# bd-iaas-us/infiniStore

Measured on AMD Instinct MI355X. Metric: put_get_GBps, higher is better.
Workload: dtype bf16; 1 GPU; model=kvcache-store, block_kb=128, global_batch=2048, seq_len=0, parallelism=shard1, client_procs=4, resident_steps=976

## Files before the change

### csrc/server/server.cpp

```cpp
#include "server.h"

#include "../core/crash.h"

#include <algorithm>
#include <chrono>
#include <cstring>
#include <future>
#include <unistd.h>

#include "../core/log.h"

namespace ifs {

namespace {

bool debug_on() {
    static const bool on = getenv("IFS_SERVER_DEBUG") != nullptr;
    return on;
}
using Clock = std::chrono::steady_clock;
double us(Clock::time_point a, Clock::time_point b) {
    return std::chrono::duration<double, std::micro>(b - a).count();
}

// ... 365 lines not shown
            conn_close(c);
            return;
        }
    } else {
        uv_tcp_init(&io->loop, &c->tcp);
        c->tcp.data = c;
        if (uv_tcp_open(&c->tcp, fd) != 0) {
            conn_close(c);
            return;
        }
        uv_tcp_nodelay(&c->tcp, 1);
    }
    io->conns.push_back(c);
    uv_read_start(
        c->stream(),
        [](uv_handle_t*, size_t suggested, uv_buf_t* buf) {
            buf->base = static_cast<char*>(malloc(suggested));
            buf->len = suggested;
        },
        [](uv_stream_t* stream, ssize_t nread, const uv_buf_t* buf) {
            auto* c = static_cast<Conn*>(stream->data);
            Server* srv = c->srv;
            if (nread < 0) {
                free(buf->base);
                auto& v = c->owner->conns;
                v.erase(std::remove(v.begin(), v.end(), c), v.end());
                srv->verbs_teardown(c);
                srv->shm_teardown(c);
                conn_close(c);
                return;
            }
            if (nread == 0) {
                free(buf->base);
                return;
            }
            c->buf.insert(c->buf.end(), reinterpret_cast<uint8_t*>(buf->base),
                          reinterpret_cast<uint8_t*>(buf->base) + nread);
            free(buf->base);
            size_t consumed = 0;
            for (;;) {
                if (c->state == Conn::kHeader) {
                    if (c->buf.size() - consumed < sizeof(Header)) break;
                    memcpy(&c->hdr, c->buf.data() + consumed, sizeof(Header));
                    consumed += sizeof(Header);
                    if (c->hdr.magic != kMagic) {
                        WARN("bad magic from client; closing");
                        auto& v = c->owner->conns;
                        v.erase(std::remove(v.begin(), v.end(), c), v.end());
                        srv->verbs_teardown(c);
                        srv->shm_teardown(c);
                        conn_close(c);
                        return;
                    }
                    size_t cap = (c->hdr.op == OP_TCP_PUT) ? (256u << 20) : kProtocolBufferSize;
                    if (c->hdr.body_size > cap) {
                        WARN("body too large (%u) for op %c", c->hdr.body_size, c->hdr.op);
                        auto& v = c->owner->conns;
                        v.erase(std::remove(v.begin(), v.end(), c), v.end());
                        srv->verbs_teardown(c);
                        srv->shm_teardown(c);
                        conn_close(c);
                        return;
                    }
                    c->state = Conn::kBody;
                }
                if (c->state == Conn::kBody) {
                    if (c->buf.size() - consumed < c->hdr.body_size) break;
                    std::vector<uint8_t> body(c->buf.data() + consumed,
                                              c->buf.data() + consumed + c->hdr.body_size);
                    consumed += c->hdr.body_size;
                    c->state = Conn::kHeader;
                    srv->handle_request(c, c->hdr.op, std::move(body));
                    if (c->closed) return;
                }
            }
            if (consumed) c->buf.erase(c->buf.begin(), c->buf.begin() + consumed);
        });
}

namespace {

Server::LocalView to_view(const LocalMetaMsg& msg) {
    Server::LocalView v;
    v.device = msg.device;
    v.pid = msg.pid;
    v.base_ptr = msg.base_ptr;
    v.base_offset = msg.base_offset;
    v.block_size = msg.block_size;
    v.ipc = msg.ipc_handle.data();
    v.ipc_len = msg.ipc_handle.size();
    v.blocks.reserve(msg.blocks.size());
    for (auto& b : msg.blocks) v.blocks.push_back({std::string_view(b.key), b.offset});
    return v;
}

bool parse_packed_local(const uint8_t* body, size_t body_len, Server::LocalView* v) {
    if (body_len < sizeof(PackedLocalHdr)) return false;
    PackedLocalHdr h;
    memcpy(&h, body, sizeof(h));
    size_t n = h.n_blocks;
    size_t off_end = sizeof(h) + n * 8;
    if (body_len < off_end) return false;
    v->device = h.device;
    v->pid = h.pid;
    v->base_ptr = h.base_ptr;
    v->base_offset = h.base_offset;
    v->block_size = h.block_size;
    v->flags = h.flags;
    v->alloc_mb = h.rsvd;
    v->ipc = body + offsetof(PackedLocalHdr, ipc);
    v->ipc_len = 64;
    const uint64_t* offs = reinterpret_cast<const uint64_t*>(body + sizeof(h));
    const char* kp = reinterpret_cast<const char*>(body + off_end);
    const char* kend = reinterpret_cast<const char*>(body + body_len);
    v->blocks.reserve(n);
    for (size_t i = 0; i < n; i++) {
        const char* nul = static_cast<const char*>(memchr(kp, 0, kend - kp));
        const char* ke = nul ? nul : kend;
        if (kp > kend || (i + 1 < n && !nul)) return false;
        v->blocks.push_back({std::string_view(kp, ke - kp), offs[i]});
        kp = nul ? nul + 1 : kend;
    }
    return true;
}

}

void Server::handle_request(Conn* c, char op, std::vector<uint8_t> body) {
    DEBUG("request op=%s body=%zu", op_name(op).c_str(), body.size());
    struct Timer {
        Server* s;
        char op;
        std::chrono::steady_clock::time_point t0 = std::chrono::steady_clock::now();
        ~Timer() {
            auto us = std::chrono::duration_cast<std::chrono::microseconds>(
                          std::chrono::steady_clock::now() - t0)
                          .count();
            auto& st = s->op_stats_[static_cast<uint8_t>(op) & 127];
            st.count.fetch_add(1, std::memory_order_relaxed);
            st.total_us.fetch_add(static_cast<uint64_t>(us), std::memory_order_relaxed);
            uint64_t prev = st.max_us.load(std::memory_order_relaxed);
            while (static_cast<uint64_t>(us) > prev &&
                   !st.max_us.compare_exchange_weak(prev, static_cast<uint64_t>(us))) {
            }
        }
    } timer{this, op};
    switch (op) {
        case OP_W: {
            LocalMetaMsg msg;
            if (!parse_local_meta(body.data(), body.size(), &msg)) return send_status(c, INVALID_REQ);
            return op_local_write(c, to_view(msg), ReqCtx{});
        }
        case OP_R: {
            LocalMetaMsg msg;
            if (!parse_local_meta(body.data(), body.size(), &msg)) return send_status(c, INVALID_REQ);
            return op_local_read(c, to_view(msg), ReqCtx{});
        }
        case OP_W_FAST: {
            LocalView v;
            if (!parse_packed_local(body.data(), body.size(), &v))
                return send_status(c, INVALID_REQ);
            return op_local_write(c, v, ReqCtx{});
        }
        case OP_R_FAST: {
            LocalView v;
            if (!parse_packed_local(body.data(), body.size(), &v))
                return send_status(c, INVALID_REQ);
            return op_local_read(c, v, ReqCtx{});
        }
        case OP_SYNC:
            return op_sync(c, ReqCtx{});
        case OP_SHM_SETUP:
            return op_shm_setup(c, body);
        case OP_RDMA_EXCHANGE:
            return op_exchange(c, body);
        case OP_RDMA_ALLOCATE: {
            RemoteMetaMsg msg;
            if (!parse_remote_meta(body.data(), body.size(), &msg))
                return send_status(c, INVALID_REQ);
            return op_allocate(c, msg);
        }
        case OP_TCP_PUT:
            return op_tcp_put(c, std::move(body));
        case OP_TCP_GET: {
            RemoteMetaMsg msg;
            if (!parse_remote_meta(body.data(), body.size(), &msg))
                return send_status(c, INVALID_REQ);
            return op_tcp_get(c, msg);
        }
        case OP_RDMA_WRITE_COMMIT: {
            RemoteMetaMsg msg;
            if (!parse_remote_meta(body.data(), body.size(), &msg))
                return send_status(c, INVALID_REQ);
            return op_commit(c, msg);
        }
        case OP_CHECK_EXIST:
            return op_check_exist(c, body, ReqCtx{});
        case OP_GET_MATCH_LAST_IDX:
            return op_match_index(c, body, ReqCtx{});
        case OP_DELETE:
            return op_delete(c, body, ReqCtx{});
        case OP_STATS: {
            std::string js = stats_json();
            return send_status_payload(c, FINISH,
                                       reinterpret_cast<const uint8_t*>(js.data()), js.size());
        }
        default:
            WARN("unknown op '%c'", op);
            return send_status(c, INVALID_REQ);
    }
}

Shard* Server::shard_for_device(int device) {
    for (auto& s : shards_)
        if (s->device() == device) return s.get();
    return shards_[static_cast<size_t>(device < 0 ? 0 : device) % shards_.size()].get();
}

Shard* Server::shard_least_used() {
    Shard* best = shards_[0].get();
    size_t best_used = SIZE_MAX;
    for (auto& s : shards_) {
        size_t used = s->used_blocks();
        if (used < best_used) {
            best_used = used;
            best = s.get();
        }
    }
    return best;
}

void Server::maybe_extend(Shard* s) {
    if (!s->need_extend()) return;
    int expect = 0;
    if (!extending_.compare_exchange_strong(expect, 1)) return;
    std::lock_guard<std::mutex> jl(extend_mu_);
    if (extend_thread_.joinable()) extend_thread_.join();
    extend_thread_ = std::thread([this, s] {
        INFO("extending pool on shard dev=%d", s->device());
        void* arena = nullptr;
        if (s->extend(&arena) && arena) {
            std::lock_guard<std::mutex> lk(vdrv_mu_);
            if (vdrv_ && !vdrv_->reg_region(arena, opt_.extend_bytes, s->on_gpu(), nullptr))
                ERROR("MR registration of extended arena failed; verbs reads from it will error");
        }
        extending_.store(0);
    });
}

namespace {
void* resolve_client_base(Server::Conn* c, const Server::LocalView& msg) {
    if (msg.pid != 0 && msg.pid == static_cast<int32_t>(getpid()) && msg.base_ptr != 0)
        return reinterpret_cast<void*>(msg.base_ptr);
    if (msg.alloc_mb >= 2048) {
        ERROR("refusing IPC import of a %u MB client allocation: "
              "hipIpcOpenMemHandle hangs for >= 2 GiB allocations under "
              "dmabuf IPC; split the tensor or use the fabric path",
              msg.alloc_mb);
        return nullptr;
    }
    std::vector<uint8_t> key(msg.ipc, msg.ipc + msg.ipc_len);
    std::lock_guard<std::mutex> lk(c->ipc_mu);
    auto it = c->ipc_cache.find(key);
    if (it != c->ipc_cache.end()) return it->second.first;
    if (c->ipc_cache.size() >= 64 && c->remain.load() == 0 &&
        c->fabric_inflight.load() == 0 && c->ipc_pin.load() == 1) {
        for (auto& kv2 : c->ipc_cache) gpu::ipc_close(kv2.second.first);
        c->ipc_cache.clear();
    }
    gpu::IpcHandle h;
    memcpy(h.bytes, msg.ipc, gpu::kIpcHandleSize);
    void* base = gpu::ipc_open(h, msg.device);
    if (base) c->ipc_cache.emplace(std::move(key), std::make_pair(base, msg.device));
    return base;
}

struct IpcPinGuard {
    Server::Conn* c;
    explicit IpcPinGuard(Server::Conn* conn) : c(conn) { c->ipc_pin.fetch_add(1); }
    ~IpcPinGuard() { c->ipc_pin.fetch_sub(1); }
};
}

void Server::op_local_write(Conn* c, const LocalView& msg, const ReqCtx& ctx) {
    const bool dbg = debug_on();
    auto p0 = Clock::now();
    if (!gpu::available()) return reply_local(c, ctx, SYSTEM_ERROR);
    if (msg.ipc_len != gpu::kIpcHandleSize || msg.block_size <= 0)
        return reply_local(c, ctx, INVALID_REQ);
    IpcPinGuard pin(c);
    void* base = resolve_client_base(c, msg);
    if (!base) return reply_local(c, ctx, INTERNAL_ERROR);
    uint8_t* client_ptr = static_cast<uint8_t*>(base) + msg.base_offset;

    Shard* shard = shard_for_device(msg.device);
    size_t page = static_cast<size_t>(msg.block_size);
    size_t nb = msg.blocks.size();
    const bool quant = (msg.flags & kLocalFlagQuantFp8) != 0;
    if (quant && (page % 16 != 0)) return reply_local(c, ctx, INVALID_REQ);
    const size_t stored = quant ? page / 2 : page;

    std::vector<uint64_t> hashes(nb);
    for (size_t i = 0; i < nb; i++) hashes[i] = KvIndex::hash_of(msg.blocks[i].first);
    std::vector<uint32_t> fresh;
    fresh.reserve(nb);
    KvIndex::SweepTimes ta, td;
    index_.for_each_batched<KvIndex::Lock::kShared>(
        nb, hashes.data(), KvIndex::rotated_start(hashes.data(), nb),
        [&](KvMap& m, size_t i) {
            if (!index_.find_live(m, msg.blocks[i].first, hashes[i]))
                fresh.push_back(static_cast<uint32_t>(i));
            return true;
        },
        dbg ? &ta : nullptr);
    if (dbg && nb > 64)
        fprintf(stderr, "[pdbg2] dedup lockwait=%.0f underlock=%.0f\n", ta.lock_wait_us,
                ta.under_lock_us);
    auto p1 = Clock::now();

    n_writes_.fetch_add(1);
    size_t n_fresh = fresh.size();
    bytes_in_.fetch_add(n_fresh * page);
    bool sync_resp = (msg.flags & kLocalFlagSyncResponse) != 0;
    if (n_fresh == 0) {
        if (ctx.shm && !sync_resp) return;
        return reply_local(c, ctx, sync_resp ? FINISH : TASK_ACCEPTED);
    }

    std::vector<std::pair<void*, int>> slots;
    slots.reserve(n_fresh);
    auto try_alloc = [&] {
        slots.clear();
        return shard->allocate(stored, n_fresh,
                               [&](void* p, int idx) { slots.push_back({p, idx}); });
    };
    bool alloc_ok = try_alloc();
    for (int attempt = 0; !alloc_ok && opt_.auto_evict && attempt < 4; attempt++) {
        if (index_.evict_lru(shard, page * n_fresh * 2) == 0) break;
        alloc_ok = try_alloc();
    }
    if (!alloc_ok) return reply_local(c, ctx, OUT_OF_MEMORY);
    auto p2 = Clock::now();

    uint64_t t = index_.tick();
    SlabBatch slab_batch(n_fresh);
    auto entries = std::make_shared<std::vector<Ref<BlockEntry>>>();
    entries->reserve(n_fresh);
    Shard::CopyJob job;
    job.bytes_per_block = page;
    job.src.reserve(n_fresh);
    job.dst.reserve(n_fresh);
    auto scales_out =
        quant ? std::make_shared<std::vector<float>>(n_fresh, 1.f) : nullptr;
    if (quant) {
        job.xform = Shard::CopyJob::Xform::kQuantBf16Fp8;
        job.scales_out = scales_out;
    }
    for (size_t i = 0; i < n_fresh; i++) {
        auto* e = slab_batch.make();
        e->ptr = slots[i].first;
        e->size = stored;
        e->pool_idx = slots[i].second;
        e->shard = shard;
        e->committed = false;
        e->fp8 = quant;
        e->born_sec = KvIndex::now_sec();
        e->last_access.store(t, std::memory_order_relaxed);
        entries->emplace_back(e);
        job.src.push_back(
            reinterpret_cast<uint64_t>(client_ptr + msg.blocks[fresh[i]].second));
        job.dst.push_back(reinterpret_cast<uint64_t>(slots[i].first));
    }
    maybe_extend(shard);

    c->remain.fetch_add(1);
    c->ref();
    auto t_start = Clock::now();
    auto won = std::make_shared<std::vector<uint8_t>>(n_fresh, 0);
    auto copy_ok = std::make_shared<std::atomic<bool>>(false);
    auto arrivals = std::make_shared<std::atomic<int>>(0);
    auto fin = [this, c, entries, won, sync_resp, ctx, scales_out, copy_ok] {
        bool ok = copy_ok->load(std::memory_order_acquire);
        if (ok) {
            for (size_t i = 0; i < entries->size(); i++)
                if ((*won)[i]) {
                    if (scales_out) (*entries)[i]->scale = (*scales_out)[i];
                    (*entries)[i]->committed = true;
                }
        } else {
            c->ref();
            c->owner->post([this, c, entries, won] {
                std::vector<Ref<BlockEntry>> winners;
                for (size_t i = 0; i < entries->size(); i++)
                    if ((*won)[i]) winners.push_back((*entries)[i]);
                index_.erase_entries(winners);
                c->unref();
            });
        }
        if (sync_resp) reply_local(c, ctx, ok ? FINISH : INTERNAL_ERROR);
        finish_task(c, !ctx.shm);
    };
    job.done = [this, c, entries, fin, ctx, copy_ok, arrivals, t_start, dbg](bool ok) {
        if (dbg && entries->size() > 64)
            fprintf(stderr, "[sdbg] write n=%zu submit->complete=%.0fus\n", entries->size(),
                    us(t_start, Clock::now()));
        copy_ok->store(ok, std::memory_order_release);
        if (ctx.shm) {
            if (arrivals->fetch_add(1, std::memory_order_acq_rel) == 1) fin();
        } else {
            c->owner->post([fin, arrivals] {
                if (arrivals->fetch_add(1, std::memory_order_acq_rel) == 1) fin();
            });
        }
    };
    if (!sync_resp && !ctx.shm) send_status(c, TASK_ACCEPTED);
    bool submitted = shard->submit_copy(std::move(job));
    auto p2b = Clock::now();

    {
        std::vector<uint64_t> fresh_hashes(n_fresh);
        for (size_t p = 0; p < n_fresh; p++) fresh_hashes[p] = hashes[fresh[p]];
        std::vector<Ref<BlockEntry>> displaced;
        index_.for_each_batched<KvIndex::Lock::kExclusive>(
            n_fresh, fresh_hashes.data(), KvIndex::rotated_start(fresh_hashes.data(), n_fresh),
            [&](KvMap& m, size_t p) {
                (*won)[p] = index_.insert_locked(m, msg.blocks[fresh[p]].first, fresh_hashes[p],
                                                 (*entries)[p], true,
                                                 &displaced);
                return true;
            },
            dbg ? &td : nullptr);
        if (dbg && n_fresh > 64)
            fprintf(stderr, "[pdbg2] insert lockwait=%.0f underlock=%.0f\n", td.lock_wait_us,
                    td.under_lock_us);
    }
    if (submitted && arrivals->fetch_add(1, std::memory_order_acq_rel) == 1) fin();
    auto p3 = Clock::now();
    if (dbg && n_fresh > 64)
        fprintf(stderr, "[pdbg] dedup=%.0f alloc=%.0f submit=%.0f insert=%.0f\n", us(p0, p1),
                us(p1, p2), us(p2, p2b), us(p2b, p3));
    if (!submitted) {
        if (sync_resp) reply_local(c, ctx, INTERNAL_ERROR);
        finish_task(c, !ctx.shm);
    }
}

void Server::op_local_read(Conn* c, const LocalView& msg, const ReqCtx& ctx) {
    if (!gpu::available()) return reply_local(c, ctx, SYSTEM_ERROR);
    if (msg.ipc_len != gpu::kIpcHandleSize || msg.block_size <= 0)
        return reply_local(c, ctx, INVALID_REQ);
    IpcPinGuard pin(c);
    void* base = resolve_client_base(c, msg);
    if (!base) return reply_local(c, ctx, INTERNAL_ERROR);
    uint8_t* client_ptr = static_cast<uint8_t*>(base) + msg.base_offset;
    size_t page = static_cast<size_t>(msg.block_size);

    auto tr0 = Clock::now();
    static const bool cross_pull = [] {
        const char* v = getenv("IFS_CROSS_COPY");
        return v && std::string(v) == "reader";
    }();
    Shard* reader_shard = nullptr;
    if (cross_pull) {
        Shard* s = shard_for_device(msg.device);
        if (s->device() == msg.device) reader_shard = s;
    }
    auto exec_shard = [&](Shard* owner) {
        return (reader_shard && owner->device() != msg.device) ? reader_shard : owner;
    };
    std::map<Shard*, Shard::CopyJob> jobs;
    std::map<Shard*, Shard::CopyJob> qjobs;
    auto held = std::make_shared<std::vector<Ref<BlockEntry>>>();
    held->reserve(msg.blocks.size());
    uint64_t read_tick = index_.tick();
    std::vector<uint64_t> hashes(msg.blocks.size());
    for (size_t i = 0; i < hashes.size(); i++) hashes[i] = KvIndex::hash_of(msg.blocks[i].first);
    int err = 0;
    index_.for_each_batched<KvIndex::Lock::kShared>(
        hashes.size(), hashes.data(), 0, [&](KvMap& m, size_t i) {
            auto& b = msg.blocks[i];
            Ref<BlockEntry>* v = index_.find_live(m, b.first, hashes[i]);
            if (!v || !(*v)->committed) {
                err = KEY_NOT_FOUND;
                return false;
            }
            BlockEntry* e = v->get();
            e->last_access.store(read_tick, std::memory_order_relaxed);
            if (e->fp8 && e->size * 2 != page) {
                err = INVALID_REQ;
                return false;
            }
            auto& job = (e->fp8 ? qjobs : jobs)[exec_shard(e->shard)];
            job.bytes_per_block = page;
            if (e->fp8) {
                job.xform = Shard::CopyJob::Xform::kDequantFp8Bf16;
                job.scales_in.push_back(e->scale);
            }
            job.src.push_back(reinterpret_cast<uint64_t>(e->ptr));
            job.dst.push_back(reinterpret_cast<uint64_t>(client_ptr + b.second));
            held->push_back(*v);
            return true;
        });
    if (err) return reply_local(c, ctx, err);
    const bool dbg = debug_on();
    auto tcol = Clock::now();
    n_reads_.fetch_add(1);
    bytes_out_.fetch_add(msg.blocks.size() * page);
    bool sync_resp = (msg.flags & kLocalFlagSyncResponse) != 0;
    if (jobs.empty() && qjobs.empty())
        return reply_local(c, ctx, sync_resp ? FINISH : TASK_ACCEPTED);

    c->remain.fetch_add(1);
    c->ref();
    auto pending =
        std::make_shared<std::atomic<int>>(static_cast<int>(jobs.size() + qjobs.size()));
    auto all_ok = std::make_shared<std::atomic<bool>>(true);
    auto submit_one = [&](Shard* shard, Shard::CopyJob& job) -> bool {
        Shard::CopyJob j = std::move(job);
        auto t_start2 = Clock::now();
        j.done = [this, c, held, pending, all_ok, sync_resp, ctx, t_start2, dbg](bool ok) {
            if (dbg && held->size() > 64)
                fprintf(stderr, "[sdbg] read n=%zu submit->complete=%.0fus\n", held->size(),
                        us(t_start2, Clock::now()));
            if (!ok) all_ok->store(false);
            if (pending->fetch_sub(1) == 1) {
                if (ctx.shm) {
                    if (sync_resp) reply_local(c, ctx, all_ok->load() ? FINISH : INTERNAL_ERROR);
                    finish_task(c, false);
                } else {
                    c->owner->post([this, c, held, all_ok, sync_resp] {
                        if (sync_resp)
                            send_status(c, all_ok->load() ? FINISH : INTERNAL_ERROR);
                        finish_task(c, true);
                    });
                }
            }
        };
        if (!shard->submit_copy(std::move(j))) {
            all_ok->store(false);
            if (pending->fetch_sub(1) == 1) {
                finish_task(c, !ctx.shm);
                reply_local(c, ctx, INTERNAL_ERROR);
                return false;
            }
        }
        return true;
    };
    for (auto& [shard, job] : jobs)
        if (!submit_one(shard, job)) return;
    for (auto& [shard, job] : qjobs)
        if (!submit_one(shard, job)) return;
    if (dbg && msg.blocks.size() > 256)
        fprintf(stderr, "[rdbg] read n=%zu collect=%.0f submit=%.0f\n", msg.blocks.size(),
                us(tr0, tcol), us(tcol, Clock::now()));
    if (!sync_resp && !ctx.shm) send_status(c, TASK_ACCEPTED);
}

void Server::op_sync(Conn* c, const ReqCtx& ctx) {
    std::lock_guard<std::mutex> lk(c->sync_mu);
    if (c->remain.load() == 0) {
        reply_query(c, ctx, 0);
    } else {
        c->sync_waiting = true;
        c->sync_ctx = ctx;
    }
}

void Server::finish_task(Conn* c, bool on_owner) {
    if (c->remain.fetch_sub(1) == 1) {
        ReqCtx ctx;
        bool respond = false;
        {
            std::lock_guard<std::mutex> lk(c->sync_mu);
            if (c->sync_waiting) {
                c->sync_waiting = false;
                respond = true;
                ctx = c->sync_ctx;
            }
        }
        if (respond) {
            if (ctx.shm || on_owner) {
                reply_query(c, ctx, 0);
            } else {
                c->ref();
                c->owner->post([this, c, ctx] {
                    reply_query(c, ctx, 0);
                    c->unref();
                });
            }
        }
    }
    c->unref();
}

void Server::reply_local(Conn* c, const ReqCtx& ctx, int code) {
    if (ctx.shm && c->shm) return c->shm->push_resp(ctx.seq, code);
    send_status(c, code);
}

void Server::reply_query(Conn* c, const ReqCtx& ctx, int value) {
    if (ctx.shm && c->shm) return c->shm->push_resp(ctx.seq, value);
    send_status_raw(c, FINISH, &value, 4);
}

void Server::ShmPeer::push_resp(uint64_t seq, int status) {
    std::lock_guard<std::mutex> lk(resp_mu);
    shmring::RespRec r{};
    r.h.len = sizeof(r);
    r.h.op = 0;
    r.h.body_len = sizeof(r) - sizeof(r.h);
    r.h.seq = seq;
    r.status = status;
    uint64_t adv = 0;
    uint8_t* dst = seg.resp->claim(sizeof(r), &adv);
    if (!dst) {
        WARN("shm resp ring full; dropping response seq=%llu",
             static_cast<unsigned long long>(seq));
        return;
    }
    memcpy(dst, &r, sizeof(r));
    seg.resp->publish(adv);
}

void Server::op_shm_setup(Conn* c, const std::vector<uint8_t>& body) {
    if (c->shm || body.empty() || body.size() > 100 || body[0] != '/')
        return send_status(c, INVALID_REQ);
    if (shm_peers_.load() >= 160) return send_status(c, SYSTEM_ERROR);
    std::string name(reinterpret_cast<const char*>(body.data()), body.size());
    auto* p = new ShmPeer();
    p->srv = this;
    p->c = c;
    if (!shmring::open_segment(name, &p->seg)) {
        delete p;
        return send_status(c, INTERNAL_ERROR);
    }
    c->shm = p;
    shm_peers_.fetch_add(1);
    c->ref();
    p->th = std::thread([this, p] { shm_poll_main(p); });
    INFO("shm ring attached (%zu bytes)", p->seg.len);
    send_status(c, FINISH);
}

void Server::shm_teardown(Conn* c) {
    if (!c->shm) return;
    c->shm->stop.store(true, std::memory_order_release);
    if (c->shm->th.joinable()) c->shm->th.join();
    shm_peers_.fetch_sub(1);
}

void Server::fast_worker_main() {
    for (;;) {
        FastWork w;
        {
            std::unique_lock<std::mutex> lk(fast_mu_);
            fast_cv_.wait(lk, [this] { return stop_requested_.load() || !fast_q_.empty(); });
            if (fast_q_.empty()) {
                if (stop_requested_.load()) return;
                continue;
            }
            w = std::move(fast_q_.front());
            fast_q_.pop_front();
        }
        run_fast(w);
    }
}

void Server::run_fast(FastWork& w) {
    ReqCtx ctx{w.seq, true};
    LocalView v;
    if (!parse_packed_local(w.body.data(), w.body.size(), &v)) {
        reply_local(w.c, ctx, INVALID_REQ);
    } else if (w.op == OP_W_FAST) {
        op_local_write(w.c, v, ctx);
    } else {
        op_local_read(w.c, v, ctx);
    }
    finish_task(w.c, false);
}

void Server::shm_poll_main(ShmPeer* p) {
    Conn* c = p->c;
    auto last_work = std::chrono::steady_clock::now();
    while (!p->stop.load(std::memory_order_acquire)) {
        uint32_t len = 0;
        uint64_t skip = 0;
        bool corrupt = false;
        const uint8_t* rec = p->seg.req->peek(&len, &skip, &corrupt);
        if (corrupt) {
            ERROR("shm req ring corrupt (invalid record header); detaching poller");
            break;
        }
        if (!rec) {
            if (std::chrono::steady_clock::now() - last_work > std::chrono::milliseconds(2)) {
                usleep(50);
            } else {
#if defined(__x86_64__)
                for (int i = 0; i < 64; i++) __builtin_ia32_pause();
#else
                std::this_thread::yield();
#endif
            }
            continue;
        }
        if (len == 0) {
            p->seg.req->consume(skip);
            continue;
        }
        shmring::RecHdr h;
        memcpy(&h, rec, sizeof(h));
        const uint8_t* body = rec + sizeof(h);
        ReqCtx ctx{h.seq, true};
        auto t0 = std::chrono::steady_clock::now();
        char op = static_cast<char>(h.op);
        if (debug_on() && h.body_len > 4096)
            fprintf(stderr, "[rdbg] op=%c pickup_wait=%uus\n", op,
                    shmring::mono_us() - h.t_push_us);
        if (h.body_len + sizeof(h) > len) {
            reply_local(c, ctx, INVALID_REQ);
        } else {
            switch (op) {
                case OP_W_FAST:
                case OP_R_FAST: {
                    size_t qlen = 0;
                    bool pool = h.body_len >= 2048 && shm_peers_.load() >= 8 &&
                                !fast_workers_.empty();
                    if (pool) {
                        std::lock_guard<std::mutex> lk(fast_mu_);
                        qlen = fast_q_.size();
                    }
                    if (pool && qlen < 8192) {
                        FastWork w;
                        w.c = c;
                        w.op = op;
                        w.seq = h.seq;
                        w.body.assign(body, body + h.body_len);
                        c->remain.fetch_add(1);
                        c->ref();
                        {
                            std::lock_guard<std::mutex> lk(fast_mu_);
                            fast_q_.push_back(std::move(w));
                        }
                        fast_cv_.notify_one();
// ... 256 lines not shown
        size_t nb = whole.block_ptrs.size();
        size_t per_seg = std::max<size_t>(1, kSegBytes / page);
        size_t n_segs = (nb + per_seg - 1) / per_seg;
        auto segs_left = std::make_shared<std::atomic<int>>(static_cast<int>(n_segs));
        for (size_t off = 0; off < nb; off += per_seg) {
            size_t take = std::min(per_seg, nb - off);
            Shard::FabricJob j;
            j.is_put = false;
            j.bytes_per_block = page;
            j.raw_host = resp;
            j.block_ptrs.assign(whole.block_ptrs.begin() + static_cast<long>(off),
                                whole.block_ptrs.begin() + static_cast<long>(off + take));
            j.host_offsets.assign(whole.host_offsets.begin() + static_cast<long>(off),
                                  whole.host_offsets.begin() + static_cast<long>(off + take));
            bool first = off == 0;
            size_t seg_start = first ? 0 : 8 + off * page;
            size_t seg_len = (first ? 8 : 0) + take * page;
            j.done = [this, c, resp, segs_left, all_ok, held_sp, seg_start,
                      seg_len](bool ok) {
                if (!ok) all_ok->store(false);
                bool last = segs_left->fetch_sub(1) == 1;
                c->ref();
                c->owner->post([this, c, resp, all_ok, seg_start, seg_len, last] {
                    if (all_ok->load()) {
                        std::shared_ptr<uint8_t[]> view(resp, resp.get() + seg_start);
                        send_raw(c, std::move(view), seg_len);
                    } else if (last) {
                        conn_close(c);
                    }
                    c->unref();
                    if (last) c->unref();
                });
            };
            shard->submit_fabric(std::move(j));
        }
        return;
    }

    for (auto& [shard, job] : jobs) {
        Shard::FabricJob j = std::move(job);
        j.raw_host = resp;
        j.done = [this, c, resp, resp_len, pending, all_ok, held_sp](bool ok) {
            if (!ok) all_ok->store(false);
            if (pending->fetch_sub(1) == 1) {
                c->owner->post([this, c, resp, resp_len, all_ok] {
                    if (all_ok->load())
                        send_raw(c, resp, resp_len);
                    else
                        send_status(c, INTERNAL_ERROR);
                    c->unref();
                });
            }
        };
        shard->submit_fabric(std::move(j));
    }
}

void Server::op_check_exist(Conn* c, const std::vector<uint8_t>& body, const ReqCtx& ctx) {
    if (body.empty()) return reply_local(c, ctx, INVALID_REQ);
    std::string key(reinterpret_cast<const char*>(body.data()), body.size());
    Ref<BlockEntry> e = index_.lookup(key, KvIndex::hash_of(key));
    reply_query(c, ctx, e && e->committed ? 0 : 1);
}

void Server::op_match_index(Conn* c, const std::vector<uint8_t>& body, const ReqCtx& ctx) {
    std::vector<std::string> keys;
    if (!parse_match_request(body.data(), body.size(), &keys) || keys.empty())
        return reply_query(c, ctx, -1);
    auto present = [&](size_t i) {
        Ref<BlockEntry> e = index_.lookup(keys[i], KvIndex::hash_of(keys[i]));
        return e && e->committed;
    };
    long left = 0, right = static_cast<long>(keys.size());
    while (left < right) {
        long mid = (left + right) / 2;
        if (present(static_cast<size_t>(mid)))
            left = mid + 1;
        else
            right = mid;
    }
    reply_query(c, ctx, static_cast<int>(left - 1));
}

void Server::op_delete(Conn* c, const std::vector<uint8_t>& body, const ReqCtx& ctx) {
    std::vector<std::string> keys;
    if (!parse_match_request(body.data(), body.size(), &keys))
        return reply_local(c, ctx, INVALID_REQ);
    std::vector<uint64_t> hashes(keys.size());
    for (size_t i = 0; i < keys.size(); i++) hashes[i] = KvIndex::hash_of(keys[i]);
    std::vector<Ref<BlockEntry>> dead;
    std::map<Shard*, std::vector<Shard::BlockFree>> by_shard;
    int n = 0;
    index_.for_each_batched<KvIndex::Lock::kExclusive>(
        keys.size(), hashes.data(), 0,
        [&](KvMap& m, size_t i) {
            Ref<BlockEntry> ref;
            if (m.extract(keys[i], &ref)) dead.emplace_back(std::move(ref));
            return true;
        },
        nullptr,
        [&] {
            n += static_cast<int>(dead.size());
            for (auto& ref : dead) {
                BlockEntry* e = ref.get();
                if (e->ref_count() == 1 && e->shard && e->ptr) {
                    by_shard[e->shard].push_back({e->ptr, e->size, e->pool_idx});
                    e->shard = nullptr;
                    e->ptr = nullptr;
                }
            }
            dead.clear();
        });
    for (auto& [shard, frees] : by_shard) shard->deallocate_bulk(frees);
    reply_local(c, ctx, n);
}

std::pair<size_t, size_t> Server::compact() {
    if (!running_.load()) return {0, 0};
    size_t moved = 0, bytes = 0;
    for (auto& shard_up : shards_) {
        Shard* shard = shard_up.get();
        std::vector<Ref<BlockEntry>> held;
        std::vector<std::pair<void*, size_t>> movable;
        index_.for_each_all_locked([&](std::string_view, Ref<BlockEntry>& val) {
            BlockEntry* e = val.get();
            if (e->shard == shard && e->committed && e->ref_count() == 1) {
                held.push_back(val);
                movable.push_back({e->ptr, e->size});
            }
        });
        if (movable.empty()) continue;
        auto moves = shard->plan_compaction(movable);
        if (moves.empty()) continue;

        std::map<size_t, Shard::CopyJob> by_size;
        for (auto& m : moves) {
            auto& j = by_size[m.size];
            j.bytes_per_block = m.size;
            j.src.push_back(reinterpret_cast<uint64_t>(m.old_ptr));
            j.dst.push_back(reinterpret_cast<uint64_t>(m.new_ptr));
        }
        bool copies_ok = true;
        for (auto& [sz, j2] : by_size) {
            std::promise<bool> cp;
            auto cf = cp.get_future();
            Shard::CopyJob jj = std::move(j2);
            jj.done = [&cp](bool ok) { cp.set_value(ok); };
            if (!shard->submit_copy(std::move(jj))) {
                cp.set_value(false);
            }
            if (!cf.get()) copies_ok = false;
        }

        std::map<void*, Shard::Move*> by_old;
        for (auto& m : moves) by_old[m.old_ptr] = &m;
        index_.for_each_all_locked([&](std::string_view, Ref<BlockEntry>& val) {
            BlockEntry* e = val.get();
            auto it = by_old.find(e->ptr);
            if (it == by_old.end() || e->shard != shard) return;
            if (!copies_ok || e->ref_count() > 2) return;
            Shard::Move* m = it->second;
            e->ptr = m->new_ptr;
            e->pool_idx = m->pool_idx;
            shard->deallocate(m->old_ptr, m->size, m->pool_idx);
            m->old_ptr = nullptr;
            moved++;
            bytes += m->size;
        });
        for (auto& m : moves)
            if (m.old_ptr != nullptr)
                shard->deallocate(m.new_ptr, m.size, m.pool_idx);
    }
    return {moved, bytes};
}

namespace {
constexpr uint64_t kSnapMagic = 0x53494653504e3150ull;
struct SnapEntryHdr {
    uint32_t key_len;
    uint32_t fp8;
    uint64_t size;
    float scale;
    uint32_t _pad;
};
}

bool Server::snapshot(const std::string& path, std::pair<size_t, size_t>* out) {
    *out = {0, 0};
    std::vector<std::pair<std::string, Ref<BlockEntry>>> pinned;
    index_.for_each_shared([&](std::string_view key, Ref<BlockEntry>& val) {
        if (val->committed && !index_.expired(val.get()))
            pinned.emplace_back(std::string(key), val);
    });
    FILE* f = fopen(path.c_str(), "wb");
    if (!f) {
        ERROR("snapshot: cannot open %s", path.c_str());
        return false;
    }
    uint64_t magic = kSnapMagic, count = pinned.size();
    bool ok = fwrite(&magic, 8, 1, f) == 1 && fwrite(&count, 8, 1, f) == 1;
    std::vector<uint8_t> buf;
    for (auto& [key, ref] : pinned) {
        if (!ok) break;
        BlockEntry* e = ref.get();
        SnapEntryHdr h{static_cast<uint32_t>(key.size()), e->fp8 ? 1u : 0u, e->size,
                       e->scale, 0};
        buf.resize(e->size);
        if (e->shard->on_gpu()) {
            if (!gpu::memcpy_d2h(buf.data(), e->ptr, e->size)) {
                ok = false;
                break;
            }
        } else {
            memcpy(buf.data(), e->ptr, e->size);
        }
        ok = fwrite(&h, sizeof(h), 1, f) == 1 && fwrite(key.data(), 1, key.size(), f) == key.size() &&
             fwrite(buf.data(), 1, e->size, f) == e->size;
        out->first++;
        out->second += e->size;
    }
    fclose(f);
    if (!ok) ERROR("snapshot: write failed at entry %zu", out->first);
    return ok;
}

bool Server::restore(const std::string& path, std::pair<size_t, size_t>* out) {
    *out = {0, 0};
    FILE* f = fopen(path.c_str(), "rb");
    if (!f) {
        ERROR("restore: cannot open %s", path.c_str());
        return false;
    }
    uint64_t magic = 0, count = 0;
    if (fread(&magic, 8, 1, f) != 1 || magic != kSnapMagic || fread(&count, 8, 1, f) != 1) {
        ERROR("restore: bad snapshot header");
        fclose(f);
        return false;
    }
    std::vector<uint8_t> buf;
    std::string key;
    bool ok = true;
    for (uint64_t i = 0; i < count && ok; i++) {
        SnapEntryHdr h{};
        if (fread(&h, sizeof(h), 1, f) != 1 || h.key_len > 4096 || h.size > (1u << 30)) {
            ok = false;
            break;
        }
        key.resize(h.key_len);
        buf.resize(h.size);
        if (fread(key.data(), 1, h.key_len, f) != h.key_len ||
            fread(buf.data(), 1, h.size, f) != h.size) {
            ok = false;
            break;
        }
        Shard* shard = shard_least_used();
        void* ptr = nullptr;
        int pool_idx = -1;
        if (!shard->allocate(h.size, 1, [&](void* p, int idx) {
                ptr = p;
                pool_idx = idx;
            })) {
            WARN("restore: pool full after %zu entries", out->first);
            break;
        }
        bool copied = shard->on_gpu() ? gpu::memcpy_h2d(ptr, buf.data(), h.size)
                                      : (memcpy(ptr, buf.data(), h.size), true);
        if (!copied) {
            shard->deallocate(ptr, h.size, pool_idx);
            ok = false;
            break;
        }
        auto* e = new BlockEntry();
        e->ptr = ptr;
        e->size = h.size;
        e->pool_idx = pool_idx;
        e->shard = shard;
        e->fp8 = h.fp8 != 0;
        e->scale = h.scale;
        e->born_sec = KvIndex::now_sec();
        e->committed = true;
        e->last_access.store(index_.tick(), std::memory_order_relaxed);
        Ref<BlockEntry> ref(e);
        if (index_.insert_if_absent(key, KvIndex::hash_of(key), ref, false)) {
            out->first++;
            out->second += h.size;
        }
    }
    fclose(f);
    return ok;
}

std::string Server::stats_json() {
    char buf[1024];
    size_t used = 0, total = 0, frag = 0;
    for (auto& s : shards_) {
        used += s->used_blocks();
        total += s->total_blocks();
        frag = std::max(frag, s->largest_free_run_bytes());
    }
    snprintf(buf, sizeof(buf),
             "{\"kv_len\": %zu, \"shards\": %zu, \"used_blocks\": %zu, \"total_blocks\": %zu, "
             "\"writes\": %llu, \"reads\": %llu, \"puts\": %llu, \"gets\": %llu, "
             "\"bytes_in\": %llu, \"bytes_out\": %llu, \"largest_free_run_bytes\": %zu, "
             "\"op_us\": {",
             kvmap_len(), shards_.size(), used, total,
             (unsigned long long)n_writes_.load(), (unsigned long long)n_reads_.load(),
             (unsigned long long)n_put_.load(), (unsigned long long)n_get_.load(),
             (unsigned long long)bytes_in_.load(), (unsigned long long)bytes_out_.load(), frag);
    std::string out(buf);
    bool first = true;
    for (int i = 0; i < 128; i++) {
        uint64_t cnt = op_stats_[i].count.load();
        if (!cnt) continue;
        char entry[160];
        snprintf(entry, sizeof(entry),
                 "%s\"%s\": {\"count\": %llu, \"avg_us\": %.1f, \"max_us\": %llu}",
                 first ? "" : ", ", op_name(static_cast<char>(i)).c_str(),
                 (unsigned long long)cnt,
                 static_cast<double>(op_stats_[i].total_us.load()) / cnt,
                 (unsigned long long)op_stats_[i].max_us.load());
        out += entry;
        first = false;
    }
    out += "}}";
    return out;
}

}
```

### csrc/server/server.h

```cpp
#pragma once

#include <uv.h>

#include <atomic>
#include <condition_variable>
#include <cstdint>
#include <functional>
#include <map>
#include <memory>
#include <mutex>
#include <string>
#include <string_view>
#include <thread>
#include <unordered_map>
#include <vector>

#include "../core/mempool.h"
#include "../core/protocol.h"
#include "../core/shm_ring.h"
#include "../core/utils.h"
#include "../fabric/verbs_fabric.h"
#include "../gpu/gpu.h"
#include "kv_index.h"
#include "shard.h"

namespace ifs {

struct ServerOptions {
    int service_port = 22345;
    size_t prealloc_bytes = 16ull << 30;
    size_t block_granule = 64 << 10;
    bool auto_extend = false;
    size_t extend_bytes = 10ull << 30;
    std::vector<int> devices;
    int cpu_shards = 1;
    int n_streams = 4;
    int io_threads = 3;
    std::string log_level = "warning";
    std::string dev_name;
    int ib_port = 1;
    std::string link_type = "Ethernet";
    bool auto_evict = false;
    int ttl_seconds = 0;
};

class Server;

class Server {
   public:
    explicit Server(const ServerOptions& opt);
    ~Server();
    Server(const Server&) = delete;
    Server& operator=(const Server&) = delete;

    bool start();
    void stop();
    bool running() const { return running_.load(); }

    size_t kvmap_len() { return index_.size(); }
    size_t purge() { return index_.clear(); }
    std::string stats_json();
    std::pair<size_t, size_t> compact();
    bool snapshot(const std::string& path, std::pair<size_t, size_t>* out);
    bool restore(const std::string& path, std::pair<size_t, size_t>* out);
    int num_shards() const { return static_cast<int>(shards_.size()); }

    struct Conn;

    struct ReqCtx {
        uint64_t seq = 0;
        bool shm = false;
    };

    struct ShmPeer {
        Server* srv = nullptr;
        Conn* c = nullptr;
        shmring::Segment seg;
        std::thread th;
        std::atomic<bool> stop{false};
        std::mutex resp_mu;
        void push_resp(uint64_t seq, int status);
    };

    struct LocalView {
        int32_t device = 0;
        int32_t pid = 0;
        uint64_t base_ptr = 0;
        uint64_t base_offset = 0;
        int64_t block_size = 0;
        uint32_t flags = 0;
        uint32_t alloc_mb = 0;
        const uint8_t* ipc = nullptr;
        size_t ipc_len = 0;
        std::vector<std::pair<std::string_view, uint64_t>> blocks;
    };

    std::vector<RemoteBlockWire> allocate_blocks(Conn* c,
                                                 const std::vector<std::string>& keys,
                                                 size_t page, int* status);
    void commit_addrs(Conn* c, const std::vector<uint64_t>& addrs);
    bool collect_read_entries(const std::vector<std::string>& keys,
                              std::vector<Ref<BlockEntry>>* out);

    struct VerbsPeer;
    bool verbs_handshake(Conn* c, const std::vector<uint8_t>& body,
                         std::vector<uint8_t>* reply);
    void verbs_teardown(Conn* c);

    struct IoLoop {
        uv_loop_t loop;
        uv_async_t post_async;
        uv_async_t stop_async;
        std::thread thread;
        std::mutex post_mu;
        std::vector<std::function<void()>> posted;
        Server* srv = nullptr;
        std::vector<Conn*> conns;
        bool is_main = false;

        void post(std::function<void()> fn);
        void start();
        void request_stop() { uv_async_send(&stop_async); }
        static void on_post(uv_async_t* h);
        static void on_stop(uv_async_t* h);
    };

   private:
    friend struct VerbsPeer;

    static void on_new_connection(uv_stream_t* server, int status);
    void adopt_fd(IoLoop* io, int fd, bool is_pipe);
    static void on_new_pipe_connection(uv_stream_t* server, int status);
    void post(std::function<void()> fn) { main_io_.post(std::move(fn)); }

    void handle_request(Conn* c, char op, std::vector<uint8_t> body);
    void op_local_write(Conn* c, const LocalView& msg, const ReqCtx& ctx);
    void op_local_read(Conn* c, const LocalView& msg, const ReqCtx& ctx);
    void op_sync(Conn* c, const ReqCtx& ctx);
    void finish_task(Conn* c, bool on_owner);
    void reply_local(Conn* c, const ReqCtx& ctx, int code);
    void reply_query(Conn* c, const ReqCtx& ctx, int value);
    void op_shm_setup(Conn* c, const std::vector<uint8_t>& body);
    void shm_teardown(Conn* c);
    void shm_poll_main(ShmPeer* p);
    std::atomic<int> shm_peers_{0};

    struct FastWork {
        Conn* c = nullptr;
        char op = 0;
        uint64_t seq = 0;
        std::vector<uint8_t> body;
    };
    std::mutex fast_mu_;
    std::condition_variable fast_cv_;
    std::deque<FastWork> fast_q_;
    std::vector<std::thread> fast_workers_;
    void fast_worker_main();
    void run_fast(FastWork& w);
    void op_exchange(Conn* c, const std::vector<uint8_t>& body);
    void op_allocate(Conn* c, const RemoteMetaMsg& msg);
    void op_tcp_put(Conn* c, std::vector<uint8_t> body);
    void op_tcp_get(Conn* c, const RemoteMetaMsg& msg);
    void op_commit(Conn* c, const RemoteMetaMsg& msg);
    void op_check_exist(Conn* c, const std::vector<uint8_t>& body, const ReqCtx& ctx);
    void op_match_index(Conn* c, const std::vector<uint8_t>& body, const ReqCtx& ctx);
    void op_delete(Conn* c, const std::vector<uint8_t>& body, const ReqCtx& ctx);

    Shard* shard_for_device(int device);
    Shard* shard_least_used();
    void maybe_extend(Shard* s);
    ServerOptions opt_;
    std::vector<std::unique_ptr<Shard>> shards_;
    std::unique_ptr<vf::Driver> vdrv_;
    std::mutex vdrv_mu_;

    IoLoop main_io_;
    std::vector<std::unique_ptr<IoLoop>> workers_;
    std::atomic<uint32_t> next_worker_{0};
    uv_tcp_t listener_;
    uv_pipe_t pipe_listener_;
    bool pipe_listening_ = false;
    std::string pipe_path_;
    std::atomic<bool> running_{false};
    std::atomic<bool> stop_requested_{false};
    std::thread ttl_thread_;
    std::mutex ttl_mu_;
    std::condition_variable ttl_cv_;

    KvIndex index_;

    std::atomic<uint64_t> n_writes_{0}, n_reads_{0}, n_put_{0}, n_get_{0};
    std::atomic<uint64_t> bytes_in_{0}, bytes_out_{0};
    std::atomic<int> extending_{0};
    std::thread extend_thread_;
    std::mutex extend_mu_;

    struct OpStat {
        std::atomic<uint64_t> count{0};
        std::atomic<uint64_t> total_us{0};
        std::atomic<uint64_t> max_us{0};
    };
    OpStat op_stats_[128];
};


struct Server::Conn : RefCounted {
    Server* srv = nullptr;
    Server::IoLoop* owner = nullptr;
    union {
        uv_tcp_t tcp;
        uv_pipe_t pipe;
    };
    bool is_pipe = false;
    uv_stream_t* stream() { return reinterpret_cast<uv_stream_t*>(&tcp); }
    uv_handle_t* handle() { return reinterpret_cast<uv_handle_t*>(&tcp); }
    Conn() : tcp{} {}
    bool closed = false;

    enum State { kHeader, kBody } state = kHeader;
    Header hdr{};
    std::vector<uint8_t> buf;

    std::atomic<int> remain{0};
    bool sync_waiting = false;

    std::mutex ipc_mu;
    std::map<std::vector<uint8_t>, std::pair<void*, int>> ipc_cache;
    std::atomic<int> ipc_pin{0};

    std::unordered_map<uint64_t, Ref<BlockEntry>> pending_rdma;
    std::atomic<int> fabric_inflight{0};
    std::vector<std::vector<uint64_t>> deferred_commits;

    Server::VerbsPeer* verbs = nullptr;

    Server::ShmPeer* shm = nullptr;
    std::mutex sync_mu;
    Server::ReqCtx sync_ctx;

    ~Conn() override {
        for (auto& kv : ipc_cache) {
            if (gpu::available()) gpu::ipc_close(kv.second.first);
        }
        if (shm) {
            shm->seg.unmap();
            delete shm;
        }
    }
};

}
```

Baseline: 2093 GB/s.

## Speculatively skip dedup lookup on local writes when a connection's recent puts were all fresh

Adds a per-connection speculation flag: when the previous write had no duplicates, the server skips the shared-lock dedup sweep over the index, allocates slots for every block, and relies on insert_locked to resolve duplicates. Losing entries are dropped in the completion callback, and speculation turns off once duplicates appear. This removes one full index pass under shared locks per put. The cost is that duplicate blocks get copied and allocated needlessly on a mispredict. The change also hoists the born timestamp out of the loop and adds stats counters.

```diff
diff --git a/csrc/server/server.cpp b/csrc/server/server.cpp
--- a/csrc/server/server.cpp
+++ b/csrc/server/server.cpp
@@ -691,61 +691,77 @@
 
     std::vector<uint64_t> hashes(nb);
     for (size_t i = 0; i < nb; i++) hashes[i] = KvIndex::hash_of(msg.blocks[i].first);
-    std::vector<uint32_t> fresh;
-    fresh.reserve(nb);
+    n_writes_.fetch_add(1);
+    bool sync_resp = (msg.flags & kLocalFlagSyncResponse) != 0;
     KvIndex::SweepTimes ta, td;
-    index_.for_each_batched<KvIndex::Lock::kShared>(
-        nb, hashes.data(), KvIndex::rotated_start(hashes.data(), nb),
-        [&](KvMap& m, size_t i) {
-            if (!index_.find_live(m, msg.blocks[i].first, hashes[i]))
-                fresh.push_back(static_cast<uint32_t>(i));
-            return true;
-        },
-        dbg ? &ta : nullptr);
-    if (dbg && nb > 64)
-        fprintf(stderr, "[pdbg2] dedup lockwait=%.0f underlock=%.0f\n", ta.lock_wait_us,
-                ta.under_lock_us);
-    auto p1 = Clock::now();
-
-    n_writes_.fetch_add(1);
-    size_t n_fresh = fresh.size();
-    bytes_in_.fetch_add(n_fresh * page);
-    bool sync_resp = (msg.flags & kLocalFlagSyncResponse) != 0;
-    if (n_fresh == 0) {
-        if (ctx.shm && !sync_resp) return;
-        return reply_local(c, ctx, sync_resp ? FINISH : TASK_ACCEPTED);
-    }
 
     std::vector<std::pair<void*, int>> slots;
-    slots.reserve(n_fresh);
-    auto try_alloc = [&] {
+    slots.reserve(nb);
+    auto try_alloc = [&](size_t count) {
         slots.clear();
-        return shard->allocate(stored, n_fresh,
+        return shard->allocate(stored, count,
                                [&](void* p, int idx) { slots.push_back({p, idx}); });
     };
-    bool alloc_ok = try_alloc();
-    for (int attempt = 0; !alloc_ok && opt_.auto_evict && attempt < 4; attempt++) {
-        if (index_.evict_lru(shard, page * n_fresh * 2) == 0) break;
-        alloc_ok = try_alloc();
-    }
-    if (!alloc_ok) return reply_local(c, ctx, OUT_OF_MEMORY);
+    const bool spec =
+        nb > 0 && c->put_speculate.load(std::memory_order_relaxed) && try_alloc(nb);
+    std::vector<uint32_t> fresh;
+    std::vector<uint64_t> fresh_hashes;
+    auto p1 = p0;
+    if (!spec) {
+        fresh.reserve(nb);
+        index_.for_each_batched<KvIndex::Lock::kShared>(
+            nb, hashes.data(), KvIndex::rotated_start(hashes.data(), nb),
+            [&](KvMap& m, size_t i) {
+                if (!index_.find_live(m, msg.blocks[i].first, hashes[i]))
+                    fresh.push_back(static_cast<uint32_t>(i));
+                return true;
+            },
+            dbg ? &ta : nullptr);
+        if (dbg && nb > 64)
+            fprintf(stderr, "[pdbg2] dedup lockwait=%.0f underlock=%.0f\n", ta.lock_wait_us,
+                    ta.under_lock_us);
+        p1 = Clock::now();
+
+        size_t n_fresh = fresh.size();
+        bytes_in_.fetch_add(n_fresh * page);
+        c->put_speculate.store(n_fresh == nb, std::memory_order_relaxed);
+        if (n_fresh == 0) {
+            if (ctx.shm && !sync_resp) return;
+            return reply_local(c, ctx, sync_resp ? FINISH : TASK_ACCEPTED);
+        }
+
+        bool alloc_ok = try_alloc(n_fresh);
+        for (int attempt = 0; !alloc_ok && opt_.auto_evict && attempt < 4; attempt++) {
+            if (index_.evict_lru(shard, page * n_fresh * 2) == 0) break;
+            alloc_ok = try_alloc(n_fresh);
+        }
+        if (!alloc_ok) return reply_local(c, ctx, OUT_OF_MEMORY);
+        fresh_hashes.resize(n_fresh);
+        for (size_t p = 0; p < n_fresh; p++) fresh_hashes[p] = hashes[fresh[p]];
+    } else {
+        n_writes_spec_.fetch_add(1, std::memory_order_relaxed);
+    }
+    const size_t n_ent = spec ? nb : fresh.size();
+    const uint64_t* ent_hashes = spec ? hashes.data() : fresh_hashes.data();
+    auto src_of = [&](size_t i) { return spec ? i : static_cast<size_t>(fresh[i]); };
     auto p2 = Clock::now();
 
     uint64_t t = index_.tick();
-    SlabBatch slab_batch(n_fresh);
+    const uint32_t born = KvIndex::now_sec();
+    SlabBatch slab_batch(n_ent);
     auto entries = std::make_shared<std::vector<Ref<BlockEntry>>>();
-    entries->reserve(n_fresh);
+    entries->reserve(n_ent);
     Shard::CopyJob job;
     job.bytes_per_block = page;
-    job.src.reserve(n_fresh);
-    job.dst.reserve(n_fresh);
+    job.src.reserve(n_ent);
+    job.dst.reserve(n_ent);
     auto scales_out =
-        quant ? std::make_shared<std::vector<float>>(n_fresh, 1.f) : nullptr;
+        quant ? std::make_shared<std::vector<float>>(n_ent, 1.f) : nullptr;
     if (quant) {
         job.xform = Shard::CopyJob::Xform::kQuantBf16Fp8;
         job.scales_out = scales_out;
     }
-    for (size_t i = 0; i < n_fresh; i++) {
+    for (size_t i = 0; i < n_ent; i++) {
         auto* e = slab_batch.make();
         e->ptr = slots[i].first;
         e->size = stored;
@@ -753,11 +769,11 @@
         e->shard = shard;
         e->committed = false;
         e->fp8 = quant;
-        e->born_sec = KvIndex::now_sec();
+        e->born_sec = born;
         e->last_access.store(t, std::memory_order_relaxed);
         entries->emplace_back(e);
         job.src.push_back(
-            reinterpret_cast<uint64_t>(client_ptr + msg.blocks[fresh[i]].second));
+            reinterpret_cast<uint64_t>(client_ptr + msg.blocks[src_of(i)].second));
         job.dst.push_back(reinterpret_cast<uint64_t>(slots[i].first));
     }
     maybe_extend(shard);
@@ -765,11 +781,13 @@
     c->remain.fetch_add(1);
     c->ref();
     auto t_start = Clock::now();
-    auto won = std::make_shared<std::vector<uint8_t>>(n_fresh, 0);
+    auto won = std::make_shared<std::vector<uint8_t>>(n_ent, 0);
     auto copy_ok = std::make_shared<std::atomic<bool>>(false);
     auto arrivals = std::make_shared<std::atomic<int>>(0);
     auto fin = [this, c, entries, won, sync_resp, ctx, scales_out, copy_ok] {
         bool ok = copy_ok->load(std::memory_order_acquire);
+        for (size_t i = 0; i < entries->size(); i++)
+            if (!(*won)[i]) (*entries)[i] = Ref<BlockEntry>();
         if (ok) {
             for (size_t i = 0; i < entries->size(); i++)
                 if ((*won)[i]) {
@@ -807,27 +825,32 @@
     auto p2b = Clock::now();
 
     {
-        std::vector<uint64_t> fresh_hashes(n_fresh);
-        for (size_t p = 0; p < n_fresh; p++) fresh_hashes[p] = hashes[fresh[p]];
         std::vector<Ref<BlockEntry>> displaced;
         index_.for_each_batched<KvIndex::Lock::kExclusive>(
-            n_fresh, fresh_hashes.data(), KvIndex::rotated_start(fresh_hashes.data(), n_fresh),
+            n_ent, ent_hashes, KvIndex::rotated_start(ent_hashes, n_ent),
             [&](KvMap& m, size_t p) {
-                (*won)[p] = index_.insert_locked(m, msg.blocks[fresh[p]].first, fresh_hashes[p],
+                (*won)[p] = index_.insert_locked(m, msg.blocks[src_of(p)].first, ent_hashes[p],
                                                  (*entries)[p], true,
                                                  &displaced);
                 return true;
             },
             dbg ? &td : nullptr);
-        if (dbg && n_fresh > 64)
+        if (dbg && n_ent > 64)
             fprintf(stderr, "[pdbg2] insert lockwait=%.0f underlock=%.0f\n", td.lock_wait_us,
                     td.under_lock_us);
     }
+    if (spec) {
+        size_t winners = 0;
+        for (uint8_t w : *won) winners += w;
+        bytes_in_.fetch_add(winners * page);
+        if (winners != n_ent) dup_blocks_copied_.fetch_add(n_ent - winners);
+        c->put_speculate.store(winners == n_ent, std::memory_order_relaxed);
+    }
     if (submitted && arrivals->fetch_add(1, std::memory_order_acq_rel) == 1) fin();
     auto p3 = Clock::now();
-    if (dbg && n_fresh > 64)
-        fprintf(stderr, "[pdbg] dedup=%.0f alloc=%.0f submit=%.0f insert=%.0f\n", us(p0, p1),
-                us(p1, p2), us(p2, p2b), us(p2b, p3));
+    if (dbg && n_ent > 64)
+        fprintf(stderr, "[pdbg] dedup=%.0f alloc=%.0f submit=%.0f insert=%.0f spec=%d\n",
+                us(p0, p1), us(p1, p2), us(p2, p2b), us(p2b, p3), spec ? 1 : 0);
     if (!submitted) {
         if (sync_resp) reply_local(c, ctx, INTERNAL_ERROR);
         finish_task(c, !ctx.shm);
@@ -1690,11 +1713,14 @@
              "{\"kv_len\": %zu, \"shards\": %zu, \"used_blocks\": %zu, \"total_blocks\": %zu, "
              "\"writes\": %llu, \"reads\": %llu, \"puts\": %llu, \"gets\": %llu, "
              "\"bytes_in\": %llu, \"bytes_out\": %llu, \"largest_free_run_bytes\": %zu, "
+             "\"writes_speculative\": %llu, \"dup_blocks_copied\": %llu, "
              "\"op_us\": {",
              kvmap_len(), shards_.size(), used, total,
              (unsigned long long)n_writes_.load(), (unsigned long long)n_reads_.load(),
              (unsigned long long)n_put_.load(), (unsigned long long)n_get_.load(),
-             (unsigned long long)bytes_in_.load(), (unsigned long long)bytes_out_.load(), frag);
+             (unsigned long long)bytes_in_.load(), (unsigned long long)bytes_out_.load(), frag,
+             (unsigned long long)n_writes_spec_.load(),
+             (unsigned long long)dup_blocks_copied_.load());
     std::string out(buf);
     bool first = true;
     for (int i = 0; i < 128; i++) {
diff --git a/csrc/server/server.h b/csrc/server/server.h
--- a/csrc/server/server.h
+++ b/csrc/server/server.h
@@ -191,6 +191,7 @@
 
     std::atomic<uint64_t> n_writes_{0}, n_reads_{0}, n_put_{0}, n_get_{0};
     std::atomic<uint64_t> bytes_in_{0}, bytes_out_{0};
+    std::atomic<uint64_t> n_writes_spec_{0}, dup_blocks_copied_{0};
     std::atomic<int> extending_{0};
     std::thread extend_thread_;
     std::mutex extend_mu_;
@@ -223,6 +224,7 @@
 
     std::atomic<int> remain{0};
     bool sync_waiting = false;
+    std::atomic<bool> put_speculate{true};
 
     std::mutex ipc_mu;
     std::map<std::vector<uint8_t>, std::pair<void*, int>> ipc_cache;
```

Result: faster. 2282 GB/s (median of 6 runs) (+9.1%).
